# nguyenngocbaocmt02/multi_agent_rl_wrsn

Measured on NVIDIA B200. Metric: agent-decisions/sec, higher is better.
Workload: dtype f64

## Files before the change

multi_agent_rl_wrsn_b200/csrc/wrsn_engine.cuh:

```cuda
#ifndef WRSN_GFIX
#error "define WRSN_GFIX before including wrsn_engine.cuh"
#endif

#undef WRSN_D
#undef WRSN_DI
#undef WRSN_NOINLINE
#undef WRSN_GSZ
#if defined(WRSN_HOST_EMU)
#define WRSN_D static inline
#define WRSN_DI static inline
#define WRSN_NOINLINE static
#else
#define WRSN_D __device__ static
#define WRSN_DI __device__ __forceinline__ static
#define WRSN_NOINLINE __device__ __noinline__ static
#endif
#if WRSN_GFIX
#define WRSN_GSZ(c) WRSN_GFIX
#else
#define WRSN_GSZ(c) ((c).G)
#endif
#undef WRSN_LEAD
#if WRSN_GFIX == 32
#define WRSN_LEAD(c) true
#else
#define WRSN_LEAD(c) ((c).tid == 0)
#endif

#undef WRSN_NPT_MAX
#if WRSN_GFIX == 32
#define WRSN_NPT_MAX 4
#else
#define WRSN_NPT_MAX 9
#endif

#undef WRSN_LDG
#if defined(WRSN_HOST_EMU)
#define WRSN_LDG(p) (*(p))
#else
#define WRSN_LDG(p) __ldg(p)
#endif

#undef WRSN_SMEM_BASE
#if defined(WRSN_HOST_EMU)
#define WRSN_SMEM_BASE wrsn_smem_host
#else
#define WRSN_SMEM_BASE (reinterpret_cast<char *>(wrsn_smem_u4))
#endif

#undef WRSN_PROF_BEGIN
#undef WRSN_PROF_END
#undef WRSN_PROFB_BEGIN
#undef WRSN_PROFB_END
#if defined(WRSN_PROF) && !defined(WRSN_HOST_EMU)
#define WRSN_PROF_T0_() const long long prof_t0_ = clock64()
#define WRSN_PROF_ADD_(c, slot) do { if ((c).tid == 0) (c).hdr[slot] += (double)(clock64() - prof_t0_); } while (0)
#else
#define WRSN_PROF_T0_() do { } while (0)
#define WRSN_PROF_ADD_(c, slot) do { } while (0)
#endif
#if defined(WRSN_PROF) && WRSN_PROF == 1
#define WRSN_PROF_BEGIN() WRSN_PROF_T0_()
#define WRSN_PROF_END(c, slot) WRSN_PROF_ADD_(c, slot)
#else
#define WRSN_PROF_BEGIN() do { } while (0)
#define WRSN_PROF_END(c, slot) do { } while (0)
// ... 66 lines not shown
    c.tid = tid; c.G = G; c.work0 = 0;
    c.N = d.N; c.T = d.T; c.M = d.M; c.W = d.W; c.Tw = d.Tw; c.Npad = d.Npad; c.n_slot = d.n_slot;
    c.scr_len = L.scr_len;
    c.hdr.off = sbase + (uint32_t)L.off[WRSN_F_HDR]; c.mc.off = sbase + (uint32_t)L.off[WRSN_F_MC]; c.proc.off = sbase + (uint32_t)L.off[WRSN_F_PROC];
    c.energy.off = sbase + (uint32_t)L.off[WRSN_F_ENERGY]; c.rr.off = sbase + (uint32_t)L.off[WRSN_F_RR]; c.cs.off = sbase + (uint32_t)L.off[WRSN_F_CS];
    c.esend.off = sbase + (uint32_t)L.off[WRSN_F_ESEND]; c.logc.off = sbase + (uint32_t)L.off[WRSN_F_LOGC];
    c.nbef.off = sbase + (uint32_t)L.off[WRSN_F_NBEF]; c.naft.off = sbase + (uint32_t)L.off[WRSN_F_NAFT];
    c.level.off = sbase + (uint32_t)L.off[WRSN_F_LEVEL]; c.parent.off = sbase + (uint32_t)L.off[WRSN_F_PARENT];
    c.status.off = sbase + (uint32_t)L.off[WRSN_F_STATUS]; c.tact.off = sbase + (uint32_t)L.off[WRSN_F_TACT]; c.conn.off = sbase + (uint32_t)L.off[WRSN_F_CONN];
    c.own.off = sbase + (uint32_t)L.s_own; c.scr0.off = sbase + (uint32_t)L.s_scr0; c.scr1.off = sbase + (uint32_t)L.s_scr1;
    c.bcast.off = sbase + (uint32_t)L.s_bcast; c.red.off = sbase + (uint32_t)L.s_red; c.par.off = sbase + (uint32_t)L.s_par; c.spec.off = sbase + (uint32_t)L.s_spec; c.exptab.off = sbase + (uint32_t)L.s_exptab; c.pairs.off = sbase + (uint32_t)L.s_pairs;
    c.logtick = (double *)(state_row + L.off[WRSN_F_LOGTICK]);
    c.ring = (double *)(state_row + L.off[WRSN_F_RING]);
    c.gscratch = state_row + L.off[WRSN_F_SCRATCH];
    {
        const double *gpar = (const double *)(scen_row + L.soff[WRSN_S_PAR]);
        for (int k = tid; k < WRSN_P_LEN; k += G) c.par[k] = gpar[k];
#if !defined(WRSN_HOST_EMU)
        for (int k = tid; k < 64; k += G) c.exptab[k] = wrsn_exp2_tab[k];
#endif
    }
    c.nx = (const double *)(scen_row + L.soff[WRSN_S_NX]);
    c.ny = (const double *)(scen_row + L.soff[WRSN_S_NY]);
    c.bs_esend = (const double *)(scen_row + L.soff[WRSN_S_BS_ESEND]);
    c.nbr_dist = (const double *)(scen_row + L.soff[WRSN_S_NBR_DIST]);
    c.nbr_esend = (const double *)(scen_row + L.soff[WRSN_S_NBR_ESEND]);
    c.nbr_ptr = (const int32_t *)(scen_row + L.soff[WRSN_S_NBR_PTR]);
    c.tgt_ptr = (const int32_t *)(scen_row + L.soff[WRSN_S_TGT_PTR]);
    c.nbr_idx = (const int32_t *)(scen_row + L.soff[WRSN_S_NBR_IDX]);
    c.tgt_idx = (const int32_t *)(scen_row + L.soff[WRSN_S_TGT_IDX]);
    c.direct = (const uint8_t *)(scen_row + L.soff[WRSN_S_DIRECT]);
}

WRSN_D void gsync(const Ctx &c) {
#if defined(WRSN_HOST_EMU)
    (void)c;
#elif WRSN_GFIX == 32
    (void)c; __syncwarp();
#else
    (void)c; __syncthreads();
#endif
}

#if !defined(WRSN_HOST_EMU)
WRSN_NOINLINE double warp_sum(double v) {
#pragma unroll
    for (int o = 16; o > 0; o >>= 1) v += __shfl_xor_sync(0xffffffffu, v, o);
    return v;
}
WRSN_NOINLINE double warp_min(double v) {
#pragma unroll
    for (int o = 16; o > 0; o >>= 1) v = fmin(v, __shfl_xor_sync(0xffffffffu, v, o));
    return v;
}
#endif

WRSN_D double red_sum(const Ctx &c, double v) {
#if defined(WRSN_HOST_EMU)
    (void)c; return v;
#elif WRSN_GFIX == 32
    (void)c; return warp_sum(v);
#else
    v = warp_sum(v);
    __syncthreads();
    if ((c.tid & 31) == 0) c.red[c.tid >> 5] = v;
    __syncthreads();
    double s = 0.0;
    for (int k = 0; k < (c.G >> 5); k++) s += c.red[k];
    return s;
#endif
}
WRSN_D double red_min(const Ctx &c, double v) {
#if defined(WRSN_HOST_EMU)
    (void)c; return v;
#elif WRSN_GFIX == 32
    (void)c; return warp_min(v);
#else
    v = warp_min(v);
    __syncthreads();
    if ((c.tid & 31) == 0) c.red[c.tid >> 5] = v;
    __syncthreads();
    double s = c.red[0];
    for (int k = 1; k < (c.G >> 5); k++) s = fmin(s, c.red[k]);
    return s;
#endif
}
WRSN_DI void red_sum2(const Ctx &c, double &a, double &b, int &buf) {
#if defined(WRSN_HOST_EMU)
    (void)c; (void)a; (void)b; (void)buf;
#else
#pragma unroll
    for (int o = 16; o > 0; o >>= 1) { a += __shfl_xor_sync(0xffffffffu, a, o); b += __shfl_xor_sync(0xffffffffu, b, o); }
#if WRSN_GFIX != 32
    double *x = c.red + 16 * buf;
    buf ^= 1;
    const int nw = c.G >> 5;
    if ((c.tid & 31) == 0) { x[2 * (c.tid >> 5)] = a; x[2 * (c.tid >> 5) + 1] = b; }
    __syncthreads();
    a = x[0]; b = x[1];
    for (int k = 1; k < nw; k++) { a += x[2 * k]; b += x[2 * k + 1]; }
#else
    (void)c; (void)buf;
#endif
#endif
}
WRSN_DI void red_sum1(const Ctx &c, double &a, int &buf) {
#if defined(WRSN_HOST_EMU)
    (void)c; (void)a; (void)buf;
#else
#pragma unroll
    for (int o = 16; o > 0; o >>= 1) a += __shfl_xor_sync(0xffffffffu, a, o);
#if WRSN_GFIX != 32
    double *x = c.red + 16 * buf;
    buf ^= 1;
    const int nw = c.G >> 5;
    if ((c.tid & 31) == 0) x[c.tid >> 5] = a;
    __syncthreads();
    a = x[0];
    for (int k = 1; k < nw; k++) a += x[k];
#else
    (void)c; (void)buf;
#endif
#endif
}
WRSN_D bool red_or_warp(int v) {
#if defined(WRSN_HOST_EMU)
    return v != 0;
#else
    return __any_sync(0xffffffffu, v != 0);
#endif
}
WRSN_D int red_or(const Ctx &c, int v) {
#if defined(WRSN_HOST_EMU)
    (void)c; return v ? 1 : 0;
#elif WRSN_GFIX == 32
    (void)c; return __any_sync(0xffffffffu, v) ? 1 : 0;
#else
    (void)c; return __syncthreads_or(v) ? 1 : 0;
#endif
}
WRSN_D void atomic_or_u32(uint32_t *p, uint32_t v) {
#if !defined(WRSN_HOST_EMU)
    atomicOr(p, v);
#else
    *p |= v;
#endif
}
WRSN_D void atomic_add_i32(int *p, int v) {
#if !defined(WRSN_HOST_EMU)
    atomicAdd(p, v);
#else
    *p += v;
#endif
}
// ... 17 lines not shown
    return __ffs((int)v) - 1;
#else
    return __builtin_ctz(v);
#endif
}
WRSN_D int wrsn_popc(uint32_t v) {
#if !defined(WRSN_HOST_EMU)
    return __popc(v);
#else
    return __builtin_popcount(v);
#endif
}

WRSN_D double div_pos(double num, double den) { return num == 0.0 ? num : num / den; }

#if !defined(WRSN_HOST_EMU)
WRSN_D double wrsn_fma(double a, double b, double c) { return __fma_rn(a, b, c); }
WRSN_D double wrsn_rcp(double d) {
    double r;
    asm("rcp.approx.ftz.f64 %0, %1;" : "=d"(r) : "d"(d));
    double e = __fma_rn(-d, r, 1.0);
    r = __fma_rn(r, e, r);
    e = __fma_rn(-d, r, 1.0);
    return __fma_rn(r, e, r);
}
WRSN_D double wrsn_rsqrt(double v) {
    double r;
    asm("rsqrt.approx.ftz.f64 %0, %1;" : "=d"(r) : "d"(v));
    double e = __fma_rn(-v, r * r, 1.0);
    r = __fma_rn(r * 0.5, e, r);
    e = __fma_rn(-v, r * r, 1.0);
    return __fma_rn(r * 0.5, e, r);
}
WRSN_DI double wrsn_exp_tab(const double *tab, double z) {
    const double t = __fma_rn(z, 92.33248261689366, 6755399441055744.0);
    const int k = __double2loint(t);
    const double r = __fma_rn(t - 6755399441055744.0, -0.010830424696249145, z);
    double p = __fma_rn(r, 1.0 / 24.0, 1.0 / 6.0);
    p = __fma_rn(p, r, 0.5);
    p = __fma_rn(p, r, 1.0);
    p = __fma_rn(p, r, 1.0);
    const double y = p * tab[k & 63];
    return __hiloint2double(__double2hiint(y) + ((k >> 6) << 20), __double2loint(y));
}
#else
WRSN_D double wrsn_fma(double a, double b, double c) { return a * b + c; }
WRSN_D double wrsn_rcp(double d) { return 1.0 / d; }
WRSN_D double wrsn_rsqrt(double v) { return 1.0 / sqrt(v); }
#endif
WRSN_DI double wrsn_exp_b(const Ctx &c, double z) {
#if defined(WRSN_HOST_EMU)
    (void)c; return exp(z);
#else
    return wrsn_exp_tab(c.exptab.ptr(), z);
#endif
}


WRSN_NOINLINE double euclid2(double ax, double ay, double bx, double by) {
    double dx = ax - bx, dy = ay - by;
    return sqrt(dx * dx + dy * dy);
}

WRSN_D double wrsn_pow2_biased(int biased) {
    uint64_t b = (uint64_t)biased << 52;
#if !defined(WRSN_HOST_EMU)
    return __longlong_as_double((long long)b);
#else
    double r; memcpy(&r, &b, 8); return r;
#endif
}
WRSN_D int wrsn_biased_exp(double e) {
#if !defined(WRSN_HOST_EMU)
    return (int)((((unsigned long long)__double_as_longlong(e)) >> 52) & 0x7ffull);
#else
    uint64_t b; memcpy(&b, &e, 8); return (int)((b >> 52) & 0x7ffull);
#endif
}
WRSN_NOINLINE double sub_chain_literal(double e, double a, int n_single, double b, int n_pair) {
    for (int k = 0; k < n_single; k++) e -= a;
    for (int k = 0; k < n_pair; k++) { e -= b; e -= a; }
    return e;
}
WRSN_D double sub_chain_fast(double e, double a, int n_single, double b, int n_pair) {
    int n_a = n_single + n_pair;
    if (n_a == 0) return e;
    int ex = wrsn_biased_exp(e);
// ... 487 lines not shown
    const bool literal = c.hdr[WRSN_H_LOG_LITERAL] != 0.0;
    const bool uni = !literal && L >= WRSN_RING && c.hdr[WRSN_H_LOG_UNIFORM] >= 10.0;
    _Pragma("unroll 1")
    for (int i = c.tid; i < N; i += WRSN_GSZ(c)) {
        if (c.status[i] != 1) continue;
        c.energy[i] = fmin(c.energy[i] + c.rr[i] * 0.5, cap);
        double lg = literal ? c.logtick[i] : c.logc[i];
        if (L < WRSN_RING) {
            c.cs[i] = (c.cs[i] * (double)L + lg) / (double)(L + 1);
            c.ring[(size_t)L * c.Npad + i] = lg;
        } else {
            double old = uni ? lg : c.ring[(size_t)head * c.Npad + i];
            c.cs[i] = div_pos(c.cs[i] * (double)L - old + lg, (double)L);
            if (!uni) c.ring[(size_t)head * c.Npad + i] = lg;
        }
    }
    gsync(c);
    if (c.tid == 0) {
        if (L < WRSN_RING) c.hdr[WRSN_H_LOG_LEN] = L + 1;
        else c.hdr[WRSN_H_LOG_HEAD] = (head + 1) % WRSN_RING;
        if (literal) { c.hdr[WRSN_H_LOG_UNIFORM] = 0.0; c.hdr[WRSN_H_LOG_LITERAL] = 0.0; }
        else if (c.hdr[WRSN_H_LOG_UNIFORM] < 1e9) c.hdr[WRSN_H_LOG_UNIFORM] += 1.0;
        c.hdr[WRSN_H_NTICKS] += 1.0;
    }
    gsync(c);
}

WRSN_D double charge_rate_to(Ctx &c, const double *m, int node) {
    double t = euclid2(c.nx[node], c.ny[node], m[WRSN_MC_X], m[WRSN_MC_Y]) + c.par[WRSN_P_MC_BETA];
    return c.par[WRSN_P_MC_ALPHA] / (t * t);
}

WRSN_NOINLINE double drain_node(double e, double rr, double es, double er, int nb, int ow, int na, double cap);
WRSN_D void catch_up_for_reward(Ctx &c, double t_reward);

WRSN_D bool reward_pairs(Ctx &c) {
    bool any = false;
    for (int a = 0; a < c.M; a++) {
        const double *m = c.mc + a * WRSN_MC_LEN;
        if (m[WRSN_MC_STATUS] == 0.0 || m[WRSN_MC_TYPE] == 0.0 || m[WRSN_MC_NCONN] == 0.0) continue;
        const uint32_t *cm = c.conn + a * c.W;
        for (int w = 0; w < c.W; w++)
            for (uint32_t bits = cm[w]; bits; bits &= bits - 1u)
                if (c.status[32 * w + wrsn_ctz(bits)] == 1) any = true;
    }
    return any;
}

#undef WRSN_EMU_MAXN
#undef WRSN_SLOT_ARR
#undef WRSN_FOR_SLOTS
#if defined(WRSN_HOST_EMU)
#define WRSN_EMU_MAXN 32768
#define WRSN_SLOT_ARR(T, name) static thread_local T name[WRSN_EMU_MAXN]
#define WRSN_FOR_SLOTS(s) for (int s = 0; s < NPT; s++)
#else
#define WRSN_SLOT_ARR(T, name) T name[NPT_T > 0 ? NPT_T : WRSN_NPT_MAX]
#define WRSN_FOR_SLOTS(s) _Pragma("unroll") for (int s = 0; s < (NPT_T > 0 ? NPT_T : NPT); s++)
#endif
#undef WRSN_FLAGS_DECL
#undef WRSN_FL_GET
#undef WRSN_FL_SET
#undef WRSN_FL_CLR
#if defined(WRSN_HOST_EMU)
#define WRSN_FLAGS_DECL(name) static thread_local uint8_t name[WRSN_EMU_MAXN]; memset(name, 0, (size_t)NPT)
#define WRSN_FL_GET(name, s) (name[s] != 0)
#define WRSN_FL_SET(name, s) (name[s] = 1)
#define WRSN_FL_CLR(name, s) (name[s] = 0)
#else
#define WRSN_FLAGS_DECL(name) uint32_t name = 0u
#define WRSN_FL_GET(name, s) (((name) >> (s)) & 1u)
#define WRSN_FL_SET(name, s) ((name) |= 1u << (s))
#define WRSN_FL_CLR(name, s) ((name) &= ~(1u << (s)))
#endif

WRSN_D int nan_payload(double d) {
#if !defined(WRSN_HOST_EMU)
    return __double2loint(d);
#else
    uint64_t b; memcpy(&b, &d, 8); return (int)(uint32_t)b;
#endif
}
WRSN_D double nan_with_payload(int slot) {
    const uint64_t b = 0x7ff8000000000000ull | (uint64_t)(uint32_t)slot;
#if !defined(WRSN_HOST_EMU)
    return __longlong_as_double((long long)b);
#else
    double r; memcpy(&r, &b, 8); return r;
#endif
}

// ... 91 lines not shown
            const double H = sp[2];
            if (book) { en = en + H; en = en < cap ? en : cap; }
            if (drain) { en = (en - sp[0]) + H; en = (en < cap ? en : cap) - sp[1]; }
            c.energy[i] = en;
        } else spec_second(c, t, book, drain);
    }
}

WRSN_NOINLINE void pairs_phase(Ctx &c, double tot, int n_pairs) {
    const int G = WRSN_GSZ(c), tid = c.tid;
    if (n_pairs > WRSN_PAIR_MAX) { if (tid < c.M) reward_incentives(c, tot); return; }
    const double thr = c.par[WRSN_P_THR], cap = c.par[WRSN_P_CAP], ab2 = c.par[WRSN_P_MC_AB2];
    const double inv_tot = wrsn_rcp(tot), inv_ab2 = wrsn_rcp(ab2);
    double *pair_term = c.pairs.ptr();
    const int *pair_ids = (const int *)(pair_term + WRSN_PAIR_MAX), *pair_seg = pair_ids + 2 * WRSN_PAIR_MAX;
    for (int p = tid; p < n_pairs; p += G) {
        const int a2 = pair_ids[2 * p], i = pair_ids[2 * p + 1];
        const double ec = c.energy[i] - c.cs[i];
        double e_with = cap;
        if (ec + ab2 > cap) e_with = fmax(ec + charge_rate_fast(c, c.mc + a2 * WRSN_MC_LEN, i), cap);
        pair_term[p] = (c.scr0[i] * inv_tot) * (e_with - (ec < thr ? ec : thr)) * inv_ab2;
    }
    gsync(c);
    for (int a2 = tid; a2 < c.M; a2 += G) {
        const int p0 = pair_seg[2 * a2], p1 = pair_seg[2 * a2 + 1];
        if (p1 > p0) {
            double incentive = 0.0;
            for (int p = p0; p < p1; p++) incentive += pair_term[p];
            c.mc[a2 * WRSN_MC_LEN + WRSN_MC_EXCL] += incentive;
        }
    }
}

#if !defined(WRSN_HOST_EMU)
typedef uint32_t saddr_t;
WRSN_DI saddr_t saddr_of(const void *p) { return (saddr_t)__cvta_generic_to_shared(p); }
WRSN_DI double lds64(saddr_t a) { double v; asm volatile("ld.shared.f64 %0, [%1];" : "=d"(v) : "r"(a)); return v; }
WRSN_DI void sts64(saddr_t a, double v) { asm volatile("st.shared.f64 [%0], %1;" :: "r"(a), "d"(v) : "memory"); }
#else
typedef size_t saddr_t;
WRSN_DI saddr_t saddr_of(const void *p) { return (saddr_t)((const char *)p - WRSN_SMEM_BASE); }
WRSN_DI double lds64(saddr_t a) { return *(const double *)(WRSN_SMEM_BASE + a); }
WRSN_DI void sts64(saddr_t a, double v) { *(double *)(WRSN_SMEM_BASE + a) = v; }
#endif

template <int NPT_T>
WRSN_NOINLINE void reward_loop(Ctx &c, int batch, int n_cycles, double t_reward, int watched, int n_spec) {
    const int N = c.N, G = WRSN_GSZ(c), tid = c.tid, M = c.M;
#if defined(WRSN_HOST_EMU)
    const int NPT = N;
#else
    const int NPT = NPT_T > 0 ? NPT_T : (N + G - 1) / G;
#endif
    const double thr = c.par[WRSN_P_THR], eps = c.par[WRSN_P_EPSENV], inv_n = c.par[WRSN_P_INVN], cap = c.par[WRSN_P_CAP];
    const double ab2 = c.par[WRSN_P_MC_AB2], inv_ab2 = wrsn_rcp(ab2);
    const double *dec = c.scr1.ptr();
    const saddr_t a_energy = saddr_of(c.energy.ptr()) + 8 * tid, a_q = saddr_of(c.scr0.ptr()) + 8 * tid;
    WRSN_SLOT_ARR(double, e); WRSN_SLOT_ARR(double, cs); WRSN_SLOT_ARR(double, d); WRSN_SLOT_ARR(double, x);
    WRSN_FLAGS_DECL(f_in); WRSN_FLAGS_DECL(f_inc); WRSN_FLAGS_DECL(f_special); WRSN_FLAGS_DECL(f_unfixed);
    int any_inc = 0, any_unfixed = 0, buf = 0;
    gsync(c);
    WRSN_FOR_SLOTS(s) {
        const int i = tid + s * G;
        const bool ok = i < N && c.status[i] != 0;
        e[s] = ok ? c.energy[i] : cap; cs[s] = ok ? c.cs[i] : 0.0; d[s] = (ok && batch) ? dec[i] : 0.0;
        if (i < N) WRSN_FL_SET(f_in, s);
        if (ok) {
            if (node_in_incentive(c, i)) { WRSN_FL_SET(f_inc, s); any_inc = 1; }
            if (batch) { WRSN_FL_SET(f_unfixed, s); any_unfixed = 1; }
            if (d[s] != d[s]) WRSN_FL_SET(f_special, s);
        }
    }
    any_inc = red_or(c, any_inc);
    double *pair_term = c.pairs.ptr();
    int *pair_ids = (int *)(pair_term + WRSN_PAIR_MAX), *pair_seg = pair_ids + 2 * WRSN_PAIR_MAX;
    if (tid == 0) {
        int np = 0;
        for (int a = 0; a < M; a++) {
            const double *m = c.mc + a * WRSN_MC_LEN;
            pair_seg[2 * a] = np;
            if (m[WRSN_MC_STATUS] != 0.0 && m[WRSN_MC_TYPE] != 0.0) {
                const uint32_t *cm = c.conn + a * c.W;
                for (int w = 0; w < c.W; w++)
                    for (uint32_t bits = cm[w]; bits; bits &= bits - 1u) {
                        const int i = 32 * w + wrsn_ctz(bits);
                        if (c.status[i] != 1) continue;
                        if (np < WRSN_PAIR_MAX) { pair_ids[2 * np] = a; pair_ids[2 * np + 1] = i; }
                        np++;
                    }
            }
            pair_seg[2 * a + 1] = np;
        }
        c.bcast[8] = np;
    }
    gsync(c);
    const int n_pairs = c.bcast[8];
    const bool listed = n_pairs <= WRSN_PAIR_MAX && n_pairs <= G && M <= G;
    const bool own_pair = listed && tid < n_pairs;
    saddr_t a_pe = 0, a_pc = 0, a_pq = 0, a_pt = 0, a_excl = 0, a_seg = 0;
    int p_node = 0, p_chg = 0, seg_n = 0;
    if (own_pair) {
        p_chg = pair_ids[2 * tid]; p_node = pair_ids[2 * tid + 1];
        a_pe = saddr_of(c.energy.ptr() + p_node); a_pc = saddr_of(c.cs.ptr() + p_node); a_pq = saddr_of(c.scr0.ptr() + p_node);
        a_pt = saddr_of(pair_term + tid);
    }
    if (listed && tid < M) {
        seg_n = pair_seg[2 * tid + 1] - pair_seg[2 * tid];
        a_seg = saddr_of(pair_term + pair_seg[2 * tid]);
        a_excl = saddr_of(c.mc.ptr() + tid * WRSN_MC_LEN + WRSN_MC_EXCL);
    }
    const bool own_spec = tid < n_spec, more_spec = n_spec > G;
    double sD1 = 0.0, sD2 = 0.0, sH = 0.0, sLo = INFINITY, sHi = -INFINITY;
    saddr_t a_spec_e = 0;
    if (own_spec) {
        const double *sp = c.spec + tid * WRSN_SPEC_LEN;
        sD1 = sp[0]; sD2 = sp[1]; sH = sp[2]; sLo = sp[3]; sHi = sp[4];
        a_spec_e = saddr_of(c.energy.ptr() + (int)sp[5]);
    }
    _Pragma("unroll 1")
    for (int j = 0; j < n_cycles; j++) {
        if (watched) { catch_up_for_reward(c, t_reward + (double)j); gsync(c); }
        if (n_spec > 0) {
            if (own_spec) {
                double en = lds64(a_spec_e);
                if (en >= sLo && en <= sHi) {
                    if (j > 0) { en = en + sH; en = en < cap ? en : cap; }
                    en = (en - sD1) + sH;
                    sts64(a_spec_e, (en < cap ? en : cap) - sD2);
                } else {
                    spec_second(c, tid, j > 0, 1);
                    const double *sp = c.spec + tid * WRSN_SPEC_LEN;
                    sD1 = sp[0]; sD2 = sp[1]; sH = sp[2]; sLo = sp[3]; sHi = sp[4];
                }
            }
            if (more_spec) { for (int t = tid + G; t < n_spec; t += G) spec_second(c, t, j > 0, 1); }
            gsync(c);
        }
        if (j > 0 && red_or_warp(any_unfixed)) {
            any_unfixed = 0;
            WRSN_FOR_SLOTS(s) {
                if (WRSN_FL_GET(f_unfixed, s)) {
                    const int i = tid + s * G;
                    const double nx = cs_step(cs[s], c.logc[i]);
                    if (nx == cs[s]) WRSN_FL_CLR(f_unfixed, s);
                    else { cs[s] = nx; any_unfixed = 1; if (WRSN_FL_GET(f_inc, s)) c.cs[i] = nx; }
                }
            }
        }
        double s1 = 0.0, s2 = 0.0;
        WRSN_FOR_SLOTS(s) {
            const double e_next = e[s] - d[s];
            e[s] = WRSN_FL_GET(f_special, s) ? lds64(a_energy + 8 * s * G) : e_next;
            x[s] = cs[s] * wrsn_rcp(e[s] - thr + eps);
            s1 += x[s]; s2 = wrsn_fma(x[s], x[s], s2);
        }
        red_sum2(c, s1, s2, buf);
        const double mean = s1 * inv_n;
        double var = wrsn_fma(s2, inv_n, -(mean * mean));
        if (!(var > 1e-3 * (mean * mean))) {
            double q = 0.0;
            WRSN_FOR_SLOTS(s) { const double u = WRSN_FL_GET(f_in, s) ? x[s] - mean : 0.0; q = wrsn_fma(u, u, q); }
            red_sum1(c, q, buf);
            var = q * inv_n;
        }
        const double a = var > 0.0 ? wrsn_rsqrt(var) : 1.0 / eps;
        double tot = 0.0;
        WRSN_FOR_SLOTS(s) {
            const double q = wrsn_exp_b(c, (x[s] - mean) * a);
            tot += WRSN_FL_GET(f_in, s) ? q : 0.0;
            if (WRSN_FL_GET(f_inc, s)) {
                sts64(a_q + 8 * s * G, q);
                if (batch && !WRSN_FL_GET(f_special, s)) sts64(a_energy + 8 * s * G, e[s]);
            }
        }
        red_sum1(c, tot, buf);
        if (WRSN_GFIX == 32) gsync(c);
        if (tot == 0.0) tot = eps;
        if (n_pairs > 0) {
            if (listed) {
                if (own_pair) {
                    const double ec = lds64(a_pe) - lds64(a_pc);
                    double e_with = cap;
                    if (ec + ab2 > cap) e_with = fmax(ec + charge_rate_fast(c, c.mc + p_chg * WRSN_MC_LEN, p_node), cap);
                    sts64(a_pt, (lds64(a_pq) * wrsn_rcp(tot)) * (e_with - (ec < thr ? ec : thr)) * inv_ab2);
                }
                gsync(c);
                if (seg_n > 0) {
                    double incentive = 0.0;
                    for (int p = 0; p < seg_n; p++) incentive += lds64(a_seg + 8 * p);
                    sts64(a_excl, lds64(a_excl) + incentive);
                }
            } else pairs_phase(c, tot, n_pairs);
        }
        if (any_inc || n_spec > 0 || watched || WRSN_GFIX != 32) gsync(c);
    }
    if (batch) {
        if (n_spec > 0) spec_phase(c, n_spec, 1, 0);
        WRSN_FOR_SLOTS(s) {
            const int i = tid + s * G;
            if (!(i < N && c.status[i] != 0)) continue;
            if (WRSN_FL_GET(f_unfixed, s)) cs[s] = cs_step(cs[s], c.logc[i]);
            c.cs[i] = cs[s];
            if (!WRSN_FL_GET(f_special, s)) c.energy[i] = e[s];
        }
        gsync(c);
    }
}

WRSN_NOINLINE void reward_cycles_any(Ctx &c, int batch, int n_cycles, double t_reward, int watched, int n_spec) {
#if defined(WRSN_HOST_EMU)
    reward_loop<0>(c, batch, batch ? n_cycles : 1, t_reward, batch ? watched : 0, batch ? n_spec : 0);
#else
    const int npt = (c.N + WRSN_GSZ(c) - 1) / WRSN_GSZ(c);
    if (!batch) { n_cycles = 1; watched = 0; n_spec = 0; }
    if (npt <= 1) reward_loop<1>(c, batch, n_cycles, t_reward, watched, n_spec);
    else if (npt <= 2) reward_loop<2>(c, batch, n_cycles, t_reward, watched, n_spec);
    else if (npt <= 4) reward_loop<4>(c, batch, n_cycles, t_reward, watched, n_spec);
    else reward_loop<0>(c, batch, n_cycles, t_reward, watched, n_spec);
#endif
}

WRSN_D void ev_update_reward(Ctx &c) {
    if (reward_pairs(c)) reward_cycles_any(c, 0, 1, 0.0, 0, 0);
}

WRSN_NOINLINE double do_fitness(Ctx &c, double *per_target ) {
    const int N = c.N;
    const double thr = c.par[WRSN_P_THR];
    double *node_t = c.scr0, *lt = c.scr1;
    WRSN_PROF_BEGIN();
    for (int i = c.tid; i < N; i += WRSN_GSZ(c)) {
        double l = 0.0;
        if (c.status[i] == 1) l = (c.cs[i] == 0.0) ? INFINITY : (c.energy[i] - thr) / c.cs[i];
        lt[i] = l;
    }
    gsync(c);
    for (int i = c.tid; i < N; i += WRSN_GSZ(c)) {
        double v = -1.0;
        if (c.status[i] == 1) {
            if (c.parent[i] == -2) v = lt[i];
            else {
                double mn = lt[i];
                int h = c.parent[i], hops = 0;
                while (h >= 0 && hops++ < N) {
                    if (c.status[h] != 1) { h = -1; break; }
                    mn = fmin(mn, lt[h]);
                    h = c.parent[h];
                }
                if (h == -2) v = mn;
            }
        }
        node_t[i] = v;
    }
    gsync(c);
    for (;;) {
        int changed = 0;
// ... 237 lines not shown
    if (n < 1 || on_grid(t_end)) return;
    gsync(c);
    if (WRSN_LEAD(c)) { slot_i(p)[WRSN_PRI_LAZY] = kind; p[WRSN_PR_TINT] = t_end; p[WRSN_PR_OWED] = 0.0; }
    gsync(c);
}

WRSN_NOINLINE double slot_catch_up_core(Ctx &c, int s, double limit, bool wake, double seq) {
    double *p = slot_of(c, s);
    double t_end;
    slot_ff(c, s, limit, FF_ALL, &t_end);
    if (!wake) return 0.0;
    const double owed = p[WRSN_PR_OWED];
    gsync(c);
    if (WRSN_LEAD(c)) {
        slot_i(p)[WRSN_PRI_LAZY] = 0;
        if (owed > 0.0) { p[WRSN_PR_KEY] = WRSN_KEY_NORMAL + (seq + owed - 1.0); p[WRSN_PR_OWED] = 0.0; }
    }
    gsync(c);
    return owed;
}
WRSN_DI void slot_catch_up(Ctx &c, Clk &k, int s, double limit, bool wake) {
    const double owed = slot_catch_up_core(c, s, limit, wake, k.seq);
    k.seq += owed; k.nev += owed;
}
WRSN_D void catch_up_many(Ctx &c, double limit, int kind) {
    bool any = false;
    for (int q = 0; q < c.n_slot; q++) any = any || slot_i(slot_of(c, q))[WRSN_PRI_LAZY] >= kind;
    if (!any) return;
    gsync(c);
    for (int q = c.tid; q < c.n_slot; q += WRSN_GSZ(c))
        if (slot_i(slot_of(c, q))[WRSN_PRI_LAZY] >= kind) { double t_end; slot_ff(c, q, limit, FF_OWN, &t_end); }
    gsync(c);
}
WRSN_D void catch_up_for_reward(Ctx &c, double t_reward) { catch_up_many(c, t_reward, 2); }

WRSN_DI void wake_lazy_all(Ctx &c, Clk &k) {
    for (int q = 0; q < c.n_slot; q++)
        if (slot_i(slot_of(c, q))[WRSN_PRI_LAZY] != 0) slot_catch_up(c, k, q, k.now, true);
}
WRSN_DI void wake_lazy_sharing(Ctx &c, Clk &k, int s, int a) {
    const uint32_t *cm = c.conn + a * c.W;
    for (int q = 0; q < c.n_slot; q++) {
        const int *qi = slot_i(slot_of(c, q));
        if (q == s || qi[WRSN_PRI_LAZY] == 0 || qi[WRSN_PRI_PC] != PC_CS_FIRE) continue;
        const uint32_t *cq = c.conn + qi[WRSN_PRI_AGENT] * c.W;
        uint32_t both = 0u;
        for (int w = 0; w < c.W; w++) both |= cm[w] & cq[w];
        if (both) slot_catch_up(c, k, q, k.now, true);
    }
}

WRSN_DI void ev_slot(Ctx &c, Clk &k, int s, double other_t) {
    double *p = slot_of(c, s);
    const int a = slot_i(p)[WRSN_PRI_AGENT];
    double *m = mc_of(c, a);
    uint32_t *cm = c.conn + (size_t)a * c.W;
    const double *par = c.par.ptr();
    const bool lead = WRSN_LEAD(c);
    for (;;) {
        const int pc = slot_i(p)[WRSN_PRI_PC];
        k.nev += 1.0;
        bool again = false;
        int nx_pc = 0, nx_prio = 0;
        double nx_delay = 0.0;
        switch (pc) {
        case PC_OP_INIT: {
            const double dx = p[WRSN_PR_PHY0], dy = p[WRSN_PR_PHY1], ct = p[WRSN_PR_PHY2];
// ... 282 lines not shown
    WRSN_PROFC_END(c, WRSN_H_PROF1, pc1);
    if (n_safe <= 0) return 0;
    const int n_spec = active ? bc[0] : 0;
    if (n_spec > WRSN_SPEC_MAX) return 0;
    const double L = (double)WRSN_RING;
    WRSN_PROFC_BEGIN(pc2);
    if (KIND != 2 && !active) {
        _Pragma("unroll 1")
        for (int i = c.tid; i < N; i += WRSN_GSZ(c)) {
            if (c.status[i] != 1) continue;
            const double dec = c.scr1[i];
            if (dec == dec) c.energy[i] = c.energy[i] - dec * (double)n_safe;
            else {
                double e_end;
                const int nb = c.nbef[i], na = c.naft[i];
                const int ow = c.parent[i] != -1 ? (int)c.own[i] : 0;
                replay_cycles(c.energy[i], c.rr[i], c.esend[i], er, nb, ow, na, thr, cap, n_safe, &e_end);
                c.energy[i] = e_end;
            }
            const double lg = c.logc[i];
            double cs = c.cs[i];
            for (int t = 0; t < n_safe; t++) {
                const double nx = div_pos(cs * L - lg + lg, L);
                if (nx == cs) break;
                cs = nx;
            }
            c.cs[i] = cs;
        }
        gsync(c);
        WRSN_PROFC_END(c, WRSN_H_PROF2, pc2);
    } else {
        int watched = 0;
        for (int q = 0; q < c.n_slot; q++) watched |= slot_i(slot_of(c, q))[WRSN_PRI_LAZY] == 2 ? 1 : 0;
        reward_cycles_any(c, 1, n_safe, t_reward, watched, n_spec);
        WRSN_PROFC_END(c, WRSN_H_PROF3, pc2);
    }
    if (c.tid == 0) {
        double *hw = c.hdr;
        hw[WRSN_H_LOG_HEAD] = (double)(((int)hw[WRSN_H_LOG_HEAD] + n_safe) % WRSN_RING);
        if (hw[WRSN_H_LOG_UNIFORM] < 1e9) hw[WRSN_H_LOG_UNIFORM] = fmin(hw[WRSN_H_LOG_UNIFORM] + (double)n_safe, 1e9);
        hw[WRSN_H_NTICKS] += (double)n_safe;
        hw[WRSN_H_NBATCH] += (double)n_safe;
    }
    gsync(c);
    WRSN_PROF_END(c, WRSN_H_PROF2);
    return n_safe + (active ? (1 << 30) : 0);
}

WRSN_DI int batch_window(Ctx &c, const Clk &k, double gt, double maxtime) {
    const double H = fmin(fmin(k.mc_t, k.until_t), maxtime - 2.0);
    const bool ur_on = k.ur_t < INFINITY, net_on = k.net_t < INFINITY;
    if (!(gt + 1.0 <= H && (!net_on || (k.net_state == 2 && k.net_t == gt + 0.5 && c.hdr[WRSN_H_ALIVE] != 0.0)) &&
          (!ur_on || (k.ur_t == gt + 0.5 && (!net_on || k.ur_key < k.net_key))))) return 0;
    const double span = fmin(H - gt, 1048576.0);
    int n = (int)span;
    while (n > 0 && !(gt + (double)n <= H)) n--;
    return n;
}
WRSN_DI void batch_commit(Clk &k, double gt, int batched) {
    const bool ur_on = k.ur_t < INFINITY, net_on = k.net_t < INFINITY;
    const double nb = (double)batched;
    const double per = 2.0 + (ur_on ? 1.0 : 0.0) + (net_on ? 2.0 : 0.0);
    double s0 = k.seq + per * (nb - 1.0);
    if (ur_on) { s0 += 1.0; k.ur_key = WRSN_KEY_NORMAL + s0; k.ur_t += nb; }
    if (net_on) { s0 += 1.0; k.net_key = WRSN_KEY_NORMAL + (s0 + 2.0); k.net_t += nb; }
    k.nodes_key = WRSN_KEY_NORMAL + (s0 + 1.0);
    k.seq += per * nb; k.nev += per * nb - 1.0;
// ... 326 lines not shown
```

Baseline: 1.358 million.

## Replace templated register-slot reward loop with shared-memory streaming loop

Removes the NPT-templated reward_loop instantiations that cached per-node energy, cs and x values in register arrays. The replacement is a single non-templated loop that streams these values from shared memory each cycle through raw ld.shared/st.shared addresses. It also converts the reductions and the exp table lookup to use shared addresses, and splits out pair-list building and the two-pass variance as noinline helpers. This is meant to cut register pressure and code size (fewer instantiations, noinline catch_up_for_reward), at the cost of extra shared-memory traffic inside the hot cycle loop.

```diff
diff --git a/multi_agent_rl_wrsn_b200/csrc/wrsn_engine.cuh b/multi_agent_rl_wrsn_b200/csrc/wrsn_engine.cuh
--- a/multi_agent_rl_wrsn_b200/csrc/wrsn_engine.cuh
+++ b/multi_agent_rl_wrsn_b200/csrc/wrsn_engine.cuh
@@ -25,13 +25,6 @@
 #define WRSN_LEAD(c) true
 #else
 #define WRSN_LEAD(c) ((c).tid == 0)
-#endif
-
-#undef WRSN_NPT_MAX
-#if WRSN_GFIX == 32
-#define WRSN_NPT_MAX 4
-#else
-#define WRSN_NPT_MAX 9
 #endif
 
 #undef WRSN_LDG
@@ -164,6 +157,18 @@
     c.direct = (const uint8_t *)(scen_row + L.soff[WRSN_S_DIRECT]);
 }
 
+#if !defined(WRSN_HOST_EMU)
+typedef uint32_t saddr_t;
+WRSN_DI saddr_t saddr_of(const void *p) { return (saddr_t)__cvta_generic_to_shared(p); }
+WRSN_DI double lds64(saddr_t a) { double v; asm volatile("ld.shared.f64 %0, [%1];" : "=d"(v) : "r"(a)); return v; }
+WRSN_DI void sts64(saddr_t a, double v) { asm volatile("st.shared.f64 [%0], %1;" :: "r"(a), "d"(v) : "memory"); }
+#else
+typedef size_t saddr_t;
+WRSN_DI saddr_t saddr_of(const void *p) { return (saddr_t)((const char *)p - WRSN_SMEM_BASE); }
+WRSN_DI double lds64(saddr_t a) { return *(const double *)(WRSN_SMEM_BASE + a); }
+WRSN_DI void sts64(saddr_t a, double v) { *(double *)(WRSN_SMEM_BASE + a) = v; }
+#endif
+
 WRSN_D void gsync(const Ctx &c) {
 #if defined(WRSN_HOST_EMU)
     (void)c;
@@ -217,41 +222,41 @@
     return s;
 #endif
 }
-WRSN_DI void red_sum2(const Ctx &c, double &a, double &b, int &buf) {
+WRSN_DI void red_sum2(saddr_t red, int tid, int G, double &a, double &b, int &buf) {
 #if defined(WRSN_HOST_EMU)
-    (void)c; (void)a; (void)b; (void)buf;
+    (void)red; (void)tid; (void)G; (void)a; (void)b; (void)buf;
 #else
 #pragma unroll
     for (int o = 16; o > 0; o >>= 1) { a += __shfl_xor_sync(0xffffffffu, a, o); b += __shfl_xor_sync(0xffffffffu, b, o); }
 #if WRSN_GFIX != 32
-    double *x = c.red + 16 * buf;
+    const saddr_t x = red + 128u * (uint32_t)buf;
     buf ^= 1;
-    const int nw = c.G >> 5;
-    if ((c.tid & 31) == 0) { x[2 * (c.tid >> 5)] = a; x[2 * (c.tid >> 5) + 1] = b; }
+    const int nw = G >> 5;
+    if ((tid & 31) == 0) { sts64(x + 16u * (uint32_t)(tid >> 5), a); sts64(x + 16u * (uint32_t)(tid >> 5) + 8u, b); }
     __syncthreads();
-    a = x[0]; b = x[1];
-    for (int k = 1; k < nw; k++) { a += x[2 * k]; b += x[2 * k + 1]; }
-#else
-    (void)c; (void)buf;
-#endif
-#endif
-}
-WRSN_DI void red_sum1(const Ctx &c, double &a, int &buf) {
+    a = lds64(x); b = lds64(x + 8u);
+    for (int k = 1; k < nw; k++) { a += lds64(x + 16u * (uint32_t)k); b += lds64(x + 16u * (uint32_t)k + 8u); }
+#else
+    (void)red; (void)tid; (void)G; (void)buf;
+#endif
+#endif
+}
+WRSN_DI void red_sum1(saddr_t red, int tid, int G, double &a, int &buf) {
 #if defined(WRSN_HOST_EMU)
-    (void)c; (void)a; (void)buf;
+    (void)red; (void)tid; (void)G; (void)a; (void)buf;
 #else
 #pragma unroll
     for (int o = 16; o > 0; o >>= 1) a += __shfl_xor_sync(0xffffffffu, a, o);
 #if WRSN_GFIX != 32
-    double *x = c.red + 16 * buf;
+    const saddr_t x = red + 128u * (uint32_t)buf;
     buf ^= 1;
-    const int nw = c.G >> 5;
-    if ((c.tid & 31) == 0) x[c.tid >> 5] = a;
+    const int nw = G >> 5;
+    if ((tid & 31) == 0) sts64(x + 8u * (uint32_t)(tid >> 5), a);
     __syncthreads();
-    a = x[0];
-    for (int k = 1; k < nw; k++) a += x[k];
-#else
-    (void)c; (void)buf;
+    a = lds64(x);
+    for (int k = 1; k < nw; k++) a += lds64(x + 8u * (uint32_t)k);
+#else
+    (void)red; (void)tid; (void)G; (void)buf;
 #endif
 #endif
 }
@@ -335,7 +340,7 @@
     e = __fma_rn(-v, r * r, 1.0);
     return __fma_rn(r * 0.5, e, r);
 }
-WRSN_DI double wrsn_exp_tab(const double *tab, double z) {
+WRSN_DI double wrsn_exp_tab(saddr_t tab, double z) {
     const double t = __fma_rn(z, 92.33248261689366, 6755399441055744.0);
     const int k = __double2loint(t);
     const double r = __fma_rn(t - 6755399441055744.0, -0.010830424696249145, z);
@@ -343,7 +348,7 @@
     p = __fma_rn(p, r, 0.5);
     p = __fma_rn(p, r, 1.0);
     p = __fma_rn(p, r, 1.0);
-    const double y = p * tab[k & 63];
+    const double y = p * lds64(tab + 8u * (uint32_t)(k & 63));
     return __hiloint2double(__double2hiint(y) + ((k >> 6) << 20), __double2loint(y));
 }
 #else
@@ -351,11 +356,11 @@
 WRSN_D double wrsn_rcp(double d) { return 1.0 / d; }
 WRSN_D double wrsn_rsqrt(double v) { return 1.0 / sqrt(v); }
 #endif
-WRSN_DI double wrsn_exp_b(const Ctx &c, double z) {
+WRSN_DI double wrsn_exp_b(saddr_t tab, double z) {
 #if defined(WRSN_HOST_EMU)
-    (void)c; return exp(z);
-#else
-    return wrsn_exp_tab(c.exptab.ptr(), z);
+    (void)tab; return exp(z);
+#else
+    return wrsn_exp_tab(tab, z);
 #endif
 }
 
@@ -909,7 +914,7 @@
 }
 
 WRSN_NOINLINE double drain_node(double e, double rr, double es, double er, int nb, int ow, int na, double cap);
-WRSN_D void catch_up_for_reward(Ctx &c, double t_reward);
+WRSN_NOINLINE void catch_up_for_reward(Ctx &c, double t_reward);
 
 WRSN_D bool reward_pairs(Ctx &c) {
     bool any = false;
@@ -925,15 +930,8 @@
 }
 
 #undef WRSN_EMU_MAXN
-#undef WRSN_SLOT_ARR
-#undef WRSN_FOR_SLOTS
 #if defined(WRSN_HOST_EMU)
 #define WRSN_EMU_MAXN 32768
-#define WRSN_SLOT_ARR(T, name) static thread_local T name[WRSN_EMU_MAXN]
-#define WRSN_FOR_SLOTS(s) for (int s = 0; s < NPT; s++)
-#else
-#define WRSN_SLOT_ARR(T, name) T name[NPT_T > 0 ? NPT_T : WRSN_NPT_MAX]
-#define WRSN_FOR_SLOTS(s) _Pragma("unroll") for (int s = 0; s < (NPT_T > 0 ? NPT_T : NPT); s++)
 #endif
 #undef WRSN_FLAGS_DECL
 #undef WRSN_FL_GET
@@ -1091,51 +1089,13 @@
     }
 }
 
-#if !defined(WRSN_HOST_EMU)
-typedef uint32_t saddr_t;
-WRSN_DI saddr_t saddr_of(const void *p) { return (saddr_t)__cvta_generic_to_shared(p); }
-WRSN_DI double lds64(saddr_t a) { double v; asm volatile("ld.shared.f64 %0, [%1];" : "=d"(v) : "r"(a)); return v; }
-WRSN_DI void sts64(saddr_t a, double v) { asm volatile("st.shared.f64 [%0], %1;" :: "r"(a), "d"(v) : "memory"); }
-#else
-typedef size_t saddr_t;
-WRSN_DI saddr_t saddr_of(const void *p) { return (saddr_t)((const char *)p - WRSN_SMEM_BASE); }
-WRSN_DI double lds64(saddr_t a) { return *(const double *)(WRSN_SMEM_BASE + a); }
-WRSN_DI void sts64(saddr_t a, double v) { *(double *)(WRSN_SMEM_BASE + a) = v; }
-#endif
-
-template <int NPT_T>
-WRSN_NOINLINE void reward_loop(Ctx &c, int batch, int n_cycles, double t_reward, int watched, int n_spec) {
-    const int N = c.N, G = WRSN_GSZ(c), tid = c.tid, M = c.M;
-#if defined(WRSN_HOST_EMU)
-    const int NPT = N;
-#else
-    const int NPT = NPT_T > 0 ? NPT_T : (N + G - 1) / G;
-#endif
-    const double thr = c.par[WRSN_P_THR], eps = c.par[WRSN_P_EPSENV], inv_n = c.par[WRSN_P_INVN], cap = c.par[WRSN_P_CAP];
-    const double ab2 = c.par[WRSN_P_MC_AB2], inv_ab2 = wrsn_rcp(ab2);
-    const double *dec = c.scr1.ptr();
-    const saddr_t a_energy = saddr_of(c.energy.ptr()) + 8 * tid, a_q = saddr_of(c.scr0.ptr()) + 8 * tid;
-    WRSN_SLOT_ARR(double, e); WRSN_SLOT_ARR(double, cs); WRSN_SLOT_ARR(double, d); WRSN_SLOT_ARR(double, x);
-    WRSN_FLAGS_DECL(f_in); WRSN_FLAGS_DECL(f_inc); WRSN_FLAGS_DECL(f_special); WRSN_FLAGS_DECL(f_unfixed);
-    int any_inc = 0, any_unfixed = 0, buf = 0;
-    gsync(c);
-    WRSN_FOR_SLOTS(s) {
-        const int i = tid + s * G;
-        const bool ok = i < N && c.status[i] != 0;
-        e[s] = ok ? c.energy[i] : cap; cs[s] = ok ? c.cs[i] : 0.0; d[s] = (ok && batch) ? dec[i] : 0.0;
-        if (i < N) WRSN_FL_SET(f_in, s);
-        if (ok) {
-            if (node_in_incentive(c, i)) { WRSN_FL_SET(f_inc, s); any_inc = 1; }
-            if (batch) { WRSN_FL_SET(f_unfixed, s); any_unfixed = 1; }
-            if (d[s] != d[s]) WRSN_FL_SET(f_special, s);
-        }
-    }
-    any_inc = red_or(c, any_inc);
+
+WRSN_NOINLINE int reward_pair_list(Ctx &c) {
     double *pair_term = c.pairs.ptr();
     int *pair_ids = (int *)(pair_term + WRSN_PAIR_MAX), *pair_seg = pair_ids + 2 * WRSN_PAIR_MAX;
-    if (tid == 0) {
+    if (c.tid == 0) {
         int np = 0;
-        for (int a = 0; a < M; a++) {
+        for (int a = 0; a < c.M; a++) {
             const double *m = c.mc + a * WRSN_MC_LEN;
             pair_seg[2 * a] = np;
             if (m[WRSN_MC_STATUS] != 0.0 && m[WRSN_MC_TYPE] != 0.0) {
@@ -1153,28 +1113,70 @@
         c.bcast[8] = np;
     }
     gsync(c);
-    const int n_pairs = c.bcast[8];
+    return c.bcast[8];
+}
+
+WRSN_NOINLINE double reward_two_pass(const Ctx &c, double mean, int buf) {
+    const int G = WRSN_GSZ(c);
+    const saddr_t a_x = saddr_of(c.scr0.ptr() + c.tid);
+    double q = 0.0;
+    for (int i = c.tid, o = 0; i < c.N; i += G, o += 8 * G) { const double u = lds64(a_x + o) - mean; q = wrsn_fma(u, u, q); }
+    red_sum1(saddr_of(c.red.ptr()), c.tid, G, q, buf);
+    return q;
+}
+
+WRSN_NOINLINE void reward_loop(Ctx &c, int batch, int n_cycles, double t_reward, int watched, int n_spec) {
+    const int N = c.N, G = WRSN_GSZ(c), tid = c.tid, M = c.M;
+#if defined(WRSN_HOST_EMU)
+    const int NPT = N;
+#endif
+    const double thr = c.par[WRSN_P_THR], eps = c.par[WRSN_P_EPSENV], inv_n = c.par[WRSN_P_INVN], cap = c.par[WRSN_P_CAP];
+    const double ab2 = c.par[WRSN_P_MC_AB2], inv_ab2 = wrsn_rcp(ab2);
+    const saddr_t a_e = saddr_of(c.energy.ptr() + tid), a_cs = saddr_of(c.cs.ptr() + tid), a_x = saddr_of(c.scr0.ptr() + tid);
+    const saddr_t a_dec = saddr_of(c.scr1.ptr() + tid), a_logc = saddr_of(c.logc.ptr() + tid);
+    const saddr_t a_tab = saddr_of(c.exptab.ptr()), a_red = saddr_of(c.red.ptr());
+    const int step = 8 * G;
+    WRSN_FLAGS_DECL(f_ok); WRSN_FLAGS_DECL(f_inc); WRSN_FLAGS_DECL(f_special); WRSN_FLAGS_DECL(f_unfixed);
+    int any_inc = 0, any_unfixed = 0, buf = 0;
+    gsync(c);
+    _Pragma("unroll 1")
+    for (int i = tid, s = 0; i < N; i += G, s++) {
+        if (c.status[i] == 0) continue;
+        WRSN_FL_SET(f_ok, s);
+        if (node_in_incentive(c, i)) { WRSN_FL_SET(f_inc, s); any_inc = 1; }
+        if (batch) {
+            WRSN_FL_SET(f_unfixed, s); any_unfixed = 1;
+            if (c.scr1[i] != c.scr1[i]) WRSN_FL_SET(f_special, s);
+        }
+    }
+    any_inc = red_or(c, any_inc);
+    const int n_pairs = reward_pair_list(c);
     const bool listed = n_pairs <= WRSN_PAIR_MAX && n_pairs <= G && M <= G;
     const bool own_pair = listed && tid < n_pairs;
     saddr_t a_pe = 0, a_pc = 0, a_pq = 0, a_pt = 0, a_excl = 0, a_seg = 0;
-    int p_node = 0, p_chg = 0, seg_n = 0;
-    if (own_pair) {
-        p_chg = pair_ids[2 * tid]; p_node = pair_ids[2 * tid + 1];
-        a_pe = saddr_of(c.energy.ptr() + p_node); a_pc = saddr_of(c.cs.ptr() + p_node); a_pq = saddr_of(c.scr0.ptr() + p_node);
-        a_pt = saddr_of(pair_term + tid);
-    }
-    if (listed && tid < M) {
-        seg_n = pair_seg[2 * tid + 1] - pair_seg[2 * tid];
-        a_seg = saddr_of(pair_term + pair_seg[2 * tid]);
-        a_excl = saddr_of(c.mc.ptr() + tid * WRSN_MC_LEN + WRSN_MC_EXCL);
+    int p_node = 0, seg_n = 0;
+    const double *p_mc = nullptr;
+    {
+        double *pair_term = c.pairs.ptr();
+        const int *pair_ids = (const int *)(pair_term + WRSN_PAIR_MAX), *pair_seg = pair_ids + 2 * WRSN_PAIR_MAX;
+        if (own_pair) {
+            p_mc = c.mc + pair_ids[2 * tid] * WRSN_MC_LEN; p_node = pair_ids[2 * tid + 1];
+            a_pe = saddr_of(c.energy.ptr() + p_node); a_pc = saddr_of(c.cs.ptr() + p_node); a_pq = saddr_of(c.scr0.ptr() + p_node);
+            a_pt = saddr_of(pair_term + tid);
+        }
+        if (listed && tid < M) {
+            seg_n = pair_seg[2 * tid + 1] - pair_seg[2 * tid];
+            a_seg = saddr_of(pair_term + pair_seg[2 * tid]);
+            a_excl = saddr_of(c.mc.ptr() + tid * WRSN_MC_LEN + WRSN_MC_EXCL);
+        }
     }
     const bool own_spec = tid < n_spec, more_spec = n_spec > G;
     double sD1 = 0.0, sD2 = 0.0, sH = 0.0, sLo = INFINITY, sHi = -INFINITY;
     saddr_t a_spec_e = 0;
+    const saddr_t a_sp = saddr_of(c.spec.ptr() + tid * WRSN_SPEC_LEN);
     if (own_spec) {
-        const double *sp = c.spec + tid * WRSN_SPEC_LEN;
-        sD1 = sp[0]; sD2 = sp[1]; sH = sp[2]; sLo = sp[3]; sHi = sp[4];
-        a_spec_e = saddr_of(c.energy.ptr() + (int)sp[5]);
+        sD1 = lds64(a_sp); sD2 = lds64(a_sp + 8); sH = lds64(a_sp + 16); sLo = lds64(a_sp + 24); sHi = lds64(a_sp + 32);
+        a_spec_e = saddr_of(c.energy.ptr() + (int)lds64(a_sp + 40));
     }
     _Pragma("unroll 1")
     for (int j = 0; j < n_cycles; j++) {
@@ -1188,51 +1190,51 @@
                     sts64(a_spec_e, (en < cap ? en : cap) - sD2);
                 } else {
                     spec_second(c, tid, j > 0, 1);
-                    const double *sp = c.spec + tid * WRSN_SPEC_LEN;
-                    sD1 = sp[0]; sD2 = sp[1]; sH = sp[2]; sLo = sp[3]; sHi = sp[4];
+                    sD1 = lds64(a_sp); sD2 = lds64(a_sp + 8); sH = lds64(a_sp + 16); sLo = lds64(a_sp + 24); sHi = lds64(a_sp + 32);
                 }
             }
-            if (more_spec) { for (int t = tid + G; t < n_spec; t += G) spec_second(c, t, j > 0, 1); }
+            if (more_spec) { _Pragma("unroll 1") for (int t = tid + G; t < n_spec; t += G) spec_second(c, t, j > 0, 1); }
             gsync(c);
         }
         if (j > 0 && red_or_warp(any_unfixed)) {
             any_unfixed = 0;
-            WRSN_FOR_SLOTS(s) {
+            _Pragma("unroll 1")
+            for (int i = tid, s = 0, o = 0; i < N; i += G, s++, o += step) {
                 if (WRSN_FL_GET(f_unfixed, s)) {
-                    const int i = tid + s * G;
-                    const double nx = cs_step(cs[s], c.logc[i]);
-                    if (nx == cs[s]) WRSN_FL_CLR(f_unfixed, s);
-                    else { cs[s] = nx; any_unfixed = 1; if (WRSN_FL_GET(f_inc, s)) c.cs[i] = nx; }
+                    const double cs = lds64(a_cs + o), nx = cs_step(cs, lds64(a_logc + o));
+                    if (nx == cs) WRSN_FL_CLR(f_unfixed, s);
+                    else { sts64(a_cs + o, nx); any_unfixed = 1; }
                 }
             }
         }
         double s1 = 0.0, s2 = 0.0;
-        WRSN_FOR_SLOTS(s) {
-            const double e_next = e[s] - d[s];
-            e[s] = WRSN_FL_GET(f_special, s) ? lds64(a_energy + 8 * s * G) : e_next;
-            x[s] = cs[s] * wrsn_rcp(e[s] - thr + eps);
-            s1 += x[s]; s2 = wrsn_fma(x[s], x[s], s2);
-        }
-        red_sum2(c, s1, s2, buf);
+        _Pragma("unroll 1")
+        for (int i = tid, s = 0, o = 0; i < N; i += G, s++, o += step) {
+            double x = 0.0;
+            if (WRSN_FL_GET(f_ok, s)) {
+                double e = lds64(a_e + o);
+                if (batch && !WRSN_FL_GET(f_special, s)) { e = e - lds64(a_dec + o); sts64(a_e + o, e); }
+                x = lds64(a_cs + o) * wrsn_rcp(e - thr + eps);
+            }
+            sts64(a_x + o, x);
+            s1 += x; s2 = wrsn_fma(x, x, s2);
+        }
+        red_sum2(a_red, tid, G, s1, s2, buf);
         const double mean = s1 * inv_n;
         double var = wrsn_fma(s2, inv_n, -(mean * mean));
         if (!(var > 1e-3 * (mean * mean))) {
-            double q = 0.0;
-            WRSN_FOR_SLOTS(s) { const double u = WRSN_FL_GET(f_in, s) ? x[s] - mean : 0.0; q = wrsn_fma(u, u, q); }
-            red_sum1(c, q, buf);
-            var = q * inv_n;
+            var = reward_two_pass(c, mean, buf) * inv_n;
+            buf ^= 1;
         }
         const double a = var > 0.0 ? wrsn_rsqrt(var) : 1.0 / eps;
         double tot = 0.0;
-        WRSN_FOR_SLOTS(s) {
-            const double q = wrsn_exp_b(c, (x[s] - mean) * a);
-            tot += WRSN_FL_GET(f_in, s) ? q : 0.0;
-            if (WRSN_FL_GET(f_inc, s)) {
-                sts64(a_q + 8 * s * G, q);
-                if (batch && !WRSN_FL_GET(f_special, s)) sts64(a_energy + 8 * s * G, e[s]);
-            }
-        }
-        red_sum1(c, tot, buf);
+        _Pragma("unroll 1")
+        for (int i = tid, s = 0, o = 0; i < N; i += G, s++, o += step) {
+            const double q = wrsn_exp_b(a_tab, (lds64(a_x + o) - mean) * a);
+            tot += q;
+            if (WRSN_FL_GET(f_inc, s)) sts64(a_x + o, q);
+        }
+        red_sum1(a_red, tid, G, tot, buf);
         if (WRSN_GFIX == 32) gsync(c);
         if (tot == 0.0) tot = eps;
         if (n_pairs > 0) {
@@ -1240,12 +1242,13 @@
                 if (own_pair) {
                     const double ec = lds64(a_pe) - lds64(a_pc);
                     double e_with = cap;
-                    if (ec + ab2 > cap) e_with = fmax(ec + charge_rate_fast(c, c.mc + p_chg * WRSN_MC_LEN, p_node), cap);
+                    if (ec + ab2 > cap) e_with = fmax(ec + charge_rate_fast(c, p_mc, p_node), cap);
                     sts64(a_pt, (lds64(a_pq) * wrsn_rcp(tot)) * (e_with - (ec < thr ? ec : thr)) * inv_ab2);
                 }
                 gsync(c);
                 if (seg_n > 0) {
                     double incentive = 0.0;
+                    _Pragma("unroll 1")
                     for (int p = 0; p < seg_n; p++) incentive += lds64(a_seg + 8 * p);
                     sts64(a_excl, lds64(a_excl) + incentive);
                 }
@@ -1255,32 +1258,15 @@
     }
     if (batch) {
         if (n_spec > 0) spec_phase(c, n_spec, 1, 0);
-        WRSN_FOR_SLOTS(s) {
-            const int i = tid + s * G;
-            if (!(i < N && c.status[i] != 0)) continue;
-            if (WRSN_FL_GET(f_unfixed, s)) cs[s] = cs_step(cs[s], c.logc[i]);
-            c.cs[i] = cs[s];
-            if (!WRSN_FL_GET(f_special, s)) c.energy[i] = e[s];
-        }
+        _Pragma("unroll 1")
+        for (int i = tid, s = 0, o = 0; i < N; i += G, s++, o += step)
+            if (WRSN_FL_GET(f_unfixed, s)) sts64(a_cs + o, cs_step(lds64(a_cs + o), lds64(a_logc + o)));
         gsync(c);
     }
 }
 
-WRSN_NOINLINE void reward_cycles_any(Ctx &c, int batch, int n_cycles, double t_reward, int watched, int n_spec) {
-#if defined(WRSN_HOST_EMU)
-    reward_loop<0>(c, batch, batch ? n_cycles : 1, t_reward, batch ? watched : 0, batch ? n_spec : 0);
-#else
-    const int npt = (c.N + WRSN_GSZ(c) - 1) / WRSN_GSZ(c);
-    if (!batch) { n_cycles = 1; watched = 0; n_spec = 0; }
-    if (npt <= 1) reward_loop<1>(c, batch, n_cycles, t_reward, watched, n_spec);
-    else if (npt <= 2) reward_loop<2>(c, batch, n_cycles, t_reward, watched, n_spec);
-    else if (npt <= 4) reward_loop<4>(c, batch, n_cycles, t_reward, watched, n_spec);
-    else reward_loop<0>(c, batch, n_cycles, t_reward, watched, n_spec);
-#endif
-}
-
 WRSN_D void ev_update_reward(Ctx &c) {
-    if (reward_pairs(c)) reward_cycles_any(c, 0, 1, 0.0, 0, 0);
+    if (reward_pairs(c)) reward_loop(c, 0, 1, 0.0, 0, 0);
 }
 
 WRSN_NOINLINE double do_fitness(Ctx &c, double *per_target ) {
@@ -1584,7 +1570,7 @@
         if (slot_i(slot_of(c, q))[WRSN_PRI_LAZY] >= kind) { double t_end; slot_ff(c, q, limit, FF_OWN, &t_end); }
     gsync(c);
 }
-WRSN_D void catch_up_for_reward(Ctx &c, double t_reward) { catch_up_many(c, t_reward, 2); }
+WRSN_NOINLINE void catch_up_for_reward(Ctx &c, double t_reward) { catch_up_many(c, t_reward, 2); }
 
 WRSN_DI void wake_lazy_all(Ctx &c, Clk &k) {
     for (int q = 0; q < c.n_slot; q++)
@@ -1933,7 +1919,7 @@
     } else {
         int watched = 0;
         for (int q = 0; q < c.n_slot; q++) watched |= slot_i(slot_of(c, q))[WRSN_PRI_LAZY] == 2 ? 1 : 0;
-        reward_cycles_any(c, 1, n_safe, t_reward, watched, n_spec);
+        reward_loop(c, 1, n_safe, t_reward, watched, n_spec);
         WRSN_PROFC_END(c, WRSN_H_PROF3, pc2);
     }
     if (c.tid == 0) {
```

Result: faster. 1.576 million (median of 6 runs) (+16.0%).
